# mitenjain/nanopore

Hardware: AMD Instinct MI355X
Metric: DP cells/sec (banded pair-HMM realign: forward + backward + posterior per cell) (higher is better)
Workload: dtype f32

## Files before the change

### nanopore_amd/csrc/npr_device.h

```cpp
#pragma once
#include <cstdint>

#include "npr_internal.h"
#include "npr_band.h"

namespace npr {

struct Task {
    int64_t x_off;
    int64_t y_off;
    int64_t band_off;
    int64_t pair_off;
    int32_t lX, lY;
    int32_t D;
    int32_t pair_cap;
    int32_t flags;
    int32_t model;
    int32_t xs, ys;
    int32_t read;
    int32_t cells_pad;
    int64_t ctl_off;
    int64_t tile_off;
    int64_t rowmask_off;
};

struct Stripe {
    int32_t X;
    int32_t K;
    int32_t df, dl;
    uint32_t row0;
    int32_t pad[3];
};

struct TaskOut {
    float tot_m;
    int32_t tot_e;
    float btot_m;
    int32_t btot_e;
    int32_t npairs;
    int32_t status;
};

struct KernelArgs {
    const Task *tasks;
    TaskOut *outs;
    int32_t *queue;
    int32_t ntasks;
    const DevModel *models;
    const uint8_t *seq;
    const int32_t *lo;
    const int32_t *n;
    const uint32_t *coff;
    const Stripe *stripes;
    const uint32_t *rowmask;
    unsigned long long *prof;
    const int64_t *region;
    const uint32_t *ctl;
    char *F;
    int64_t slot_stride;
    int32_t slot_base;
    int32_t *px;
    int32_t *py;
    float *pp;
    float threshold;
    int32_t wcap;
    float *Bv;
    int32_t *Be;
    float *ring;
    float *Fx;
    double *em_T;
    double *em_E;
};

constexpr int EM_BINS = 32;

struct CompactArgs {
    const Task *tasks;
    const TaskOut *outs;
    const int64_t *dst_off;
    int32_t ntasks;
    const int32_t *px;
    const int32_t *py;
    const float *pp;
    int32_t *cx;
    int32_t *cy;
    float *cp;
};

int launch_generic(const KernelArgs &a, int grid, int threads, size_t lds_bytes, bool dense, bool global_ring, void *stream);
int launch_em(const KernelArgs &a, int grid, size_t lds_bytes, bool global_ring, void *stream);
size_t em_extra_lds_bytes();
int launch_compact(const CompactArgs &a, void *stream);
int launch_stair(const KernelArgs &a, int R, int grid, void *stream);
int launch_wide(const KernelArgs &a, int R, int NW, int grid, void *stream);
int launch_em_stair(const KernelArgs &a, int R, int grid, void *stream);
size_t em_stair_lds_bytes();
struct MeaArgs {
    const Task *tasks;
    const TaskOut *outs;
    int32_t ntasks, n_reads;
    const int32_t *px, *py;
    const float *pp;
    const int64_t *rx_off;
    const int64_t *ry_off;
    const int64_t *rp_off;
    int32_t *cnt, *start, *colsum;
    int32_t *sx, *sy, *sq, *back;
    int32_t *kx, *ky, *kq, *kback;
    int4 *vrec;
    int32_t *kept;
    const int32_t *np, *poff, *pboff, *lane_read, *lane_piece;
    int32_t *pb, *pbest;
    int32_t n_pieces;
    int32_t *best_who;
    int32_t *read_flag;
    double gap_gamma, match_gamma;
    int32_t ring;
    const int32_t *order;
    const int32_t *read_first, *read_ntasks, *task_of;
    int32_t sort_lds_bytes;
    int32_t sort_threads;
    int32_t any_global_sort;
    const int64_t *cnt_off;
    int32_t ring_only;
    int32_t *ops_tmp;
    const int64_t *ot_off;
    int32_t *n_ops, *chain_len;
    int64_t *chain_mass;
    uint32_t *ops_dense;
    const int64_t *od_off;
    int32_t *max_run;
    uint16_t *ops_dense16;
};
int launch_tile(const KernelArgs &a, int R, int NW, int grid, void *stream, bool flat = false);
size_t tile_lds_bytes(int nw);
int64_t tile_scratch_cells(int64_t rows, int R);
struct PlanSeg {
    int64_t point_first;
    int64_t band_off;
    int32_t pieces, lX, lY, pad;
};
struct SegSummary {
    int64_t cells;
    int64_t generic_cells;
    int32_t max_width;
    int32_t bad;
    int32_t rough;
    int32_t pad;
};
constexpr int kSchedClasses = 7;
constexpr int kSchedR[kSchedClasses] = {1, 2, 4, 2, 2, 4, 4};
constexpr int kSchedNW[kSchedClasses] = {1, 1, 1, 4, 8, 8, 12};
struct PlanArgs {
    int32_t n_segs, fixed_mode, width;
    const PlanPoint *points;
    const PlanSeg *segs;
    int32_t *lo, *n;
    SegSummary *summary;
};
struct SchedArgs {
    int32_t n_segs;
    const PlanSeg *segs;
    const SegSummary *summary;
    const int32_t *lo, *n;
    const int64_t *ctl_off;
    const uint32_t *cand;
    uint32_t *ctl;
    int32_t *cls;
    int64_t *cells;
};
struct StripeArgs {
    int32_t count, R;
    const int32_t *seg_index;
    const PlanSeg *segs;
    const SegSummary *summary;
    const int32_t *lo, *n;
    const int64_t *tile_off;
    Stripe *stripes;
    int64_t *rows;
};
struct CoffArgs {
    int32_t n_segs;
    const PlanSeg *segs;
    const int32_t *n;
    uint32_t *coff;
};
int launch_plan_bands(const PlanArgs &a, void *stream);
template <int R>
NPR_HD constexpr uint32_t row_bias() { return R == 4 ? 2048u : 1024u; }
NPR_HD constexpr bool stair_fits(int64_t rows, int slots) { return rows * slots < (int64_t(1) << 29) - 512; }
// ... 228 lines not shown
```

### nanopore_amd/csrc/npr_finish.cpp

```cpp
#include "npr_api_internal.h"

namespace npr_impl {

static int32_t grow_pinned(npr_ctx *ctx, void *&p, size_t &have, size_t bytes, const char *what) {
    if (bytes <= have) return NPR_OK;
    if (p) (void)hipHostFree(p);
    p = nullptr, have = 0;
    const hipError_t e = hipHostMalloc(&p, bytes + bytes / 4, hipHostMallocDefault);
    if (e != hipSuccess) return fail(ctx, NPR_ERR_NOMEM, what, e);
    have = bytes + bytes / 4;
    return NPR_OK;
}
int32_t grow_pin_pairs(npr_ctx *ctx, size_t bytes, const char *what) { return grow_pinned(ctx, ctx->pin_pairs, ctx->pin_pairs_bytes, bytes, what); }
int32_t grow_pin_stage(npr_ctx *ctx, size_t bytes, const char *what) { return grow_pinned(ctx, ctx->pin_stage, ctx->pin_stage_bytes, bytes, what); }

int32_t fetch_pieced(npr_ctx *ctx, const PiecedFetch &f) {
    if (f.count <= 0) return NPR_OK;
    const int32_t grown = grow_pin_pairs(ctx, f.elem * static_cast<size_t>(f.count), f.what_pin);
    if (grown != NPR_OK) return grown;
    constexpr int64_t kMaxPieces = 48;
    const int64_t pieces = std::min(kMaxPieces, (f.count + f.per_piece - 1) / f.per_piece);
    const int64_t piece = ((f.count + pieces - 1) / pieces + f.round_to - 1) / f.round_to * f.round_to;
    while (static_cast<int64_t>(ctx->ops_events.size()) < pieces) {
        hipEvent_t ev;
// ... 142 lines not shown
                if (len > 0) out[0] = static_cast<int32_t>(x), out[1] = static_cast<int32_t>(y), out[2] = len, out += 3;
                x += len, y += len;
            } else if (op == NPR_OP_I) {
                y += len;
            } else {
                x += len;
            }
        }
    });
    tm.lap("runs");
    DevBuf<int64_t> d_run_off;
    DevBuf<int32_t> d_runs;
    hipError_t e;
    if ((e = d_run_off.alloc_from(ctx, n + 1)) != hipSuccess || (e = b->d_rs_gx_off.alloc_from(ctx, n + 1)) != hipSuccess ||
        (e = d_runs.alloc_from(ctx, std::max<size_t>(3 * static_cast<size_t>(run_off[n]), 1))) != hipSuccess ||
        (e = b->d_rs_gy.alloc_from(ctx, std::max<int64_t>(gx_off[n], 1))) != hipSuccess)
        return fail(ctx, NPR_ERR_NOMEM, "npr_batch_create: hipMalloc (rescore tables)", e);
    HIP_TRY(ctx, hipMemcpyAsync(d_run_off.p, run_off.data(), sizeof(int64_t) * (n + 1), hipMemcpyHostToDevice, ctx->stream));
    HIP_TRY(ctx, hipMemcpyAsync(b->d_rs_gx_off.p, gx_off.data(), sizeof(int64_t) * (n + 1), hipMemcpyHostToDevice, ctx->stream));
    if (run_bytes) HIP_TRY(ctx, hipMemcpyAsync(d_runs.p, runs, run_bytes, hipMemcpyHostToDevice, ctx->stream));
    HIP_TRY(ctx, hipMemsetAsync(b->d_rs_gy.p, 0xff, sizeof(int32_t) * std::max<int64_t>(gx_off[n], 1), ctx->stream));
    RescoreArgs ra{static_cast<int32_t>(n), 0, d_run_off.p, d_runs.p, b->d_rs_gx_off.p, b->d_rs_gy.p, nullptr, nullptr, nullptr, nullptr, nullptr, nullptr, shift};
    const int rc = launch_rescore_table(ra, ctx->stream);
    if (rc != 0) return fail(ctx, NPR_ERR_HIP, "k_rescore_table launch", static_cast<hipError_t>(rc));
    HIP_TRY(ctx, hipStreamSynchronize(ctx->stream));
    tm.lap("table");
    b->rs_shift = shift, b->rs_staged = true;
    return NPR_OK;
}

int32_t rescore_sum(npr_batch *b, std::vector<double> &score) {
    npr_ctx *ctx = b->ctx;
    const int64_t n = b->n_reads, ntasks = static_cast<int64_t>(b->tasks.size());
    DevBuf<unsigned long long> d_sum;
    hipError_t e;
    if ((e = d_sum.alloc_from(ctx, n)) != hipSuccess) return fail(ctx, NPR_ERR_NOMEM, "npr_batch_finish: hipMalloc (rescore sums)", e);
    HIP_TRY(ctx, hipMemsetAsync(d_sum.p, 0, sizeof(unsigned long long) * n, ctx->stream));
    RescoreArgs ra{static_cast<int32_t>(n), static_cast<int32_t>(ntasks), nullptr, nullptr, b->d_rs_gx_off.p, b->d_rs_gy.p, b->d_tasks.p, b->d_outs.p,
                   b->d_px.p, b->d_py.p, b->d_pp.p, d_sum.p, b->rs_shift};
    const int rc = launch_rescore_sum(ra, ctx->stream);
    if (rc != 0) return fail(ctx, NPR_ERR_HIP, "k_rescore_sum launch", static_cast<hipError_t>(rc));
    std::vector<unsigned long long> sum(n);
    HIP_TRY(ctx, hipMemcpyAsync(sum.data(), d_sum.p, sizeof(unsigned long long) * n, hipMemcpyDeviceToHost, ctx->stream));
    HIP_TRY(ctx, hipStreamSynchronize(ctx->stream));
    score.assign(n, 0.0);
    for (int64_t i = 0; i < n; ++i)
        if (b->rs_columns[i] > 0) score[i] = std::ldexp(static_cast<double>(sum[i]), -b->rs_shift) / static_cast<double>(b->rs_columns[i]);
    return NPR_OK;
}


constexpr int32_t kHostStage = 1;

struct MeaPlan {
    int64_t n = 0, total = 0, n_pieces = 0;
    size_t ntask_map = 0, n_cnt = 1;
    int64_t span = 0;
    bool sort_in_lds = true;
    std::vector<int64_t> offs;
    int64_t stride() const { return n + 1; }
    int64_t *arr(int k) { return offs.data() + k * stride(); }
    int64_t cols() const { return offs[2 * stride() - 1]; }
    int64_t ops_bound() const { return offs[4 * stride() - 1]; }
    std::vector<int32_t> order;
    std::vector<int32_t> pieces_head;
};

constexpr int64_t kOffArrays = 5, kSortedArrays = 8, kSmallArrays = 6, kVrecWords = 4;

MeaPlan plan_mea(const npr_batch *b) {
    MeaPlan p;
    const int64_t n = p.n = b->n_reads;
    p.offs.assign(kOffArrays * p.stride(), 0);
    int64_t *const rx = p.arr(0), *const ry = p.arr(1), *const rp = p.arr(2), *const ot = p.arr(3), *const cnt_off = p.arr(4);
    for (int64_t i = 0; i < n; ++i) {
        const bool ok = b->results[i].status == NPR_OK;
        const int64_t lX = ok ? b->ref_len[i] : 0, lY = ok ? b->read_len[i] : 0, np = ok ? b->pair_off[i + 1] - b->pair_off[i] : 0;
        rx[i + 1] = rx[i] + lX + 1;
        ry[i + 1] = ry[i] + lY;
        rp[i + 1] = rp[i] + np;
        ot[i + 1] = ot[i] + 3 * std::min({np, lX, lY}) + 2;
    }
    p.total = rp[n];
    const int64_t lds_span = b->ctx->opt[NPR_OPT_MEA_GLOBAL_SORT] != 0 ? 0 : 16 * 1024;
    int64_t cnt_total = 0;
    for (int64_t i = 0; i < n; ++i) {
        const int64_t sp = std::max(rx[i + 1] - rx[i], ry[i + 1] - ry[i]);
        cnt_off[i] = -1;
        if (sp <= lds_span) p.span = std::max(p.span, sp);
        else cnt_off[i] = cnt_total, cnt_total += rx[i + 1] - rx[i];
    }
    cnt_off[n] = -1;
    p.sort_in_lds = cnt_total == 0;
    p.n_cnt = p.sort_in_lds ? 1 : static_cast<size_t>(cnt_total);
    p.ntask_map = b->task_of.size();
    p.order.resize(n);
    std::iota(p.order.begin(), p.order.end(), 0);
    std::stable_sort(p.order.begin(), p.order.end(), [&](int32_t x, int32_t y) { return rp[x + 1] - rp[x] > rp[y + 1] - rp[y]; });
    constexpr int64_t kMaxPieces = 64, kLanesWanted = 64 * 5 * 256;
    const int64_t kPiecePairs = std::min<int64_t>(2048, std::max<int64_t>(128, p.total / kLanesWanted));
    std::vector<int32_t> np(n);
    for (int64_t i = 0; i < n; ++i) np[i] = static_cast<int32_t>(std::min(kMaxPieces, std::max<int64_t>(1, (rp[i + 1] - rp[i] + kPiecePairs - 1) / kPiecePairs))), p.n_pieces += np[i];
    p.pieces_head.resize(3 * n + 2 * p.n_pieces);
    int32_t *const t_np = p.pieces_head.data(), *const t_poff = t_np + n, *const t_pboff = t_poff + n, *const t_lr = t_pboff + n, *const t_lp = t_lr + p.n_pieces;
    int64_t at = 0;
    for (int64_t k = 0; k < n; ++k) {
        const int32_t r = p.order[k];
        t_np[r] = np[r], t_poff[r] = static_cast<int32_t>(at), t_pboff[r] = static_cast<int32_t>(at + k);
        for (int32_t j = 0; j < np[r]; ++j) t_lr[at + j] = r, t_lp[at + j] = j;
        at += np[r];
    }
    return p;
}

static_assert(kSortedArrays % kVrecWords == 0, "vrec starts on a 16-byte boundary of m.sorted (the arena's tables start 256-byte aligned)");
inline int64_t sorted_stride(const MeaPlan &p) { return p.total + 1; }

template <typename F>
hipError_t for_each_table(MeaScratch &m, const MeaPlan &p, F &&f) {
    hipError_t e = hipSuccess;
    auto one = [&](auto &buf, int64_t count) {
        if (e == hipSuccess) e = f(buf, static_cast<size_t>(count));
    };
    one(m.off, kOffArrays * p.stride());
    one(m.mass, p.n);
    one(m.od, p.n + 1);
    one(m.cnt, p.n_cnt);
    one(m.start, p.n_cnt);
    one(m.col, p.cols() + 1);
    one(m.sorted, kSortedArrays * sorted_stride(p) + kVrecWords * (p.total + 2));
    one(m.small, kSmallArrays * p.n);
    one(m.tmp, 2 * p.ops_bound());
    one(m.map, 3 * p.n + p.ntask_map);
    one(m.dense, p.ops_bound());
    one(m.pieces, 4 * p.n_pieces + 4 * p.n);
    return e;
}

inline size_t table_align(size_t bytes) { return (bytes + 255) & ~size_t(255); }

int32_t carve_tables(npr_ctx *ctx, MeaScratch &m, const MeaPlan &p, size_t need) {
    if (poison_byte() >= 0) {
        HIP_TRY(ctx, hipStreamSynchronize(ctx->stream));
        poison(ctx->arena->F, need);
    }
    char *cur = ctx->arena->F;
    (void)for_each_table(m, p, [&](auto &buf, size_t count) {
        using T = std::remove_pointer_t<decltype(buf.p)>;
        buf.borrow(reinterpret_cast<T *>(cur), count);
        cur += table_align(sizeof(T) * count);
        return hipSuccess;
    });
    return NPR_OK;
}

int32_t obtain_tables(npr_ctx *ctx, MeaScratch &m, const MeaPlan &p, std::unique_lock<std::mutex> &arena_lock) {
    size_t need = 0;
    (void)for_each_table(m, p, [&](auto &buf, size_t count) { return need += table_align(sizeof(*buf.p) * count), hipSuccess; });
    auto arena_fits = [&] { return ctx->arena->F && need <= static_cast<size_t>(ctx->arena->cells.load()) * 8; };
    const bool fits = arena_fits();
    if (!ctx->overlap && fits) return carve_tables(ctx, m, p, need);
    if (for_each_table(m, p, [](auto &buf, size_t count) { return buf.reserve(count); }) == hipSuccess) return NPR_OK;
    (void)hipGetLastError();
    if (!(ctx->overlap && fits)) return kHostStage;
    (void)for_each_table(m, p, [](auto &buf, size_t) { return buf.release(), hipSuccess; });
    ctx->cache_flush();
    arena_lock.lock();
    if (!arena_fits()) return kHostStage;
    ++ctx->arena->epoch;
    return carve_tables(ctx, m, p, need);
}

int32_t upload_tables(npr_batch *b, const MeaPlan &p, MeaScratch &m, MeaArgs &a) {
    npr_ctx *ctx = b->ctx;
    const int64_t n = p.n, P = p.n_pieces, so = p.stride(), ss = sorted_stride(p);
    a.tasks = b->d_tasks.p, a.outs = b->d_outs.p, a.ntasks = static_cast<int32_t>(b->tasks.size()), a.n_reads = static_cast<int32_t>(n);
    a.px = b->d_px.p, a.py = b->d_py.p, a.pp = b->d_pp.p;
    a.rx_off = m.off.p, a.ry_off = m.off.p + so, a.rp_off = m.off.p + 2 * so, a.ot_off = m.off.p + 3 * so, a.cnt_off = m.off.p + 4 * so;
    a.cnt = m.cnt.p, a.start = m.start.p, a.colsum = m.col.p;
    a.sx = m.sorted.p, a.sy = m.sorted.p + ss, a.sq = m.sorted.p + 2 * ss, a.back = m.sorted.p + 3 * ss;
    a.kx = m.sorted.p + 4 * ss, a.ky = m.sorted.p + 5 * ss, a.kq = m.sorted.p + 6 * ss, a.kback = m.sorted.p + 7 * ss;
    a.vrec = reinterpret_cast<int4 *>(m.sorted.p + kSortedArrays * ss);
    a.best_who = m.small.p, a.read_flag = m.small.p + n, a.n_ops = m.small.p + 2 * n, a.chain_len = m.small.p + 3 * n, a.kept = m.small.p + 4 * n, a.max_run = m.small.p + 5 * n;
    a.chain_mass = m.mass.p;
    int32_t *const read_first = m.map.p, *const read_ntasks = read_first + n, *const task_of = read_ntasks + n, *const order = task_of + p.ntask_map;
    a.read_first = read_first, a.read_ntasks = read_ntasks, a.task_of = task_of, a.order = order;
    int32_t *const lanes = m.pieces.p + 3 * n;
    a.np = m.pieces.p, a.poff = m.pieces.p + n, a.pboff = m.pieces.p + 2 * n, a.lane_read = lanes, a.lane_piece = lanes + P, a.pbest = lanes + 2 * P, a.pb = lanes + 3 * P;
    a.n_pieces = static_cast<int32_t>(P);
    a.ops_tmp = m.tmp.p, a.od_off = m.od.p;
    a.gap_gamma = b->params.gap_gamma, a.match_gamma = b->params.match_gamma;
    a.ring = 8192;
    a.ring_only = ctx->opt[NPR_OPT_MEA_RING_ONLY] != 0 ? 1 : 0;
    a.sort_lds_bytes = static_cast<int32_t>(4 * p.span);
    a.sort_threads = ctx->overlap == 1 ? 512 : 0;
    a.any_global_sort = p.sort_in_lds ? 0 : 1;
    HIP_TRY(ctx, hipMemcpyAsync(read_first, b->read_first_task.data(), sizeof(int32_t) * n, hipMemcpyHostToDevice, ctx->stream));
    HIP_TRY(ctx, hipMemcpyAsync(read_ntasks, b->read_ntasks.data(), sizeof(int32_t) * n, hipMemcpyHostToDevice, ctx->stream));
    HIP_TRY(ctx, hipMemcpyAsync(task_of, b->task_of.data(), sizeof(int32_t) * p.ntask_map, hipMemcpyHostToDevice, ctx->stream));
    HIP_TRY(ctx, hipMemcpyAsync(order, p.order.data(), sizeof(int32_t) * n, hipMemcpyHostToDevice, ctx->stream));
    HIP_TRY(ctx, hipMemcpyAsync(m.pieces.p, p.pieces_head.data(), sizeof(int32_t) * p.pieces_head.size(), hipMemcpyHostToDevice, ctx->stream));
    HIP_TRY(ctx, hipMemcpyAsync(m.off.p, p.offs.data(), m.off.bytes(), hipMemcpyHostToDevice, ctx->stream));
    HIP_TRY(ctx, hipMemsetAsync(m.small.p, 0, m.small.bytes(), ctx->stream));
    return NPR_OK;
}

int32_t run_chain(npr_ctx *ctx, const MeaArgs &a, MeaScratch &m, std::vector<int32_t> &small, std::vector<int64_t> &mass) {
    int rc = launch_mea_sort(a, ctx->stream);
    if (rc == 0) rc = launch_mea_chain(a, ctx->stream);
    if (rc != 0) return fail(ctx, NPR_ERR_HIP, "MEA kernel launch", static_cast<hipError_t>(rc));
    small.resize(m.small.count), mass.resize(m.mass.count);
    HIP_TRY(ctx, hipMemcpyAsync(small.data(), m.small.p, m.small.bytes(), hipMemcpyDeviceToHost, ctx->stream));
    HIP_TRY(ctx, hipMemcpyAsync(mass.data(), m.mass.p, m.mass.bytes(), hipMemcpyDeviceToHost, ctx->stream));
    HIP_TRY(ctx, hipStreamSynchronize(ctx->stream));
    return NPR_OK;
}

int32_t collect_results(npr_batch *b, const std::vector<int32_t> &small, const std::vector<int64_t> &mass, int32_t &longest) {
    const int64_t n = b->n_reads;
    const int32_t *flag = small.data() + n, *nops = small.data() + 2 * n, *clen = small.data() + 3 * n, *max_run = small.data() + 5 * n;
    for (int64_t i = 0; i < n; ++i)
        if (b->results[i].status == NPR_OK && flag[i] == NPR_ERR_CAPACITY) return kHostStage;
    std::vector<int64_t> &od = b->ops_off;
    od.assign(n + 1, 0);
    longest = 0;
    for (int64_t i = 0; i < n; ++i) {
        npr_read_result &r = b->results[i];
        if (r.status == NPR_OK && flag[i] != 0) r.status = flag[i];
        const int64_t k = r.status == NPR_OK ? nops[i] : 0;
        od[i + 1] = od[i] + k;
        if (k) longest = std::max(longest, max_run[i]);
        r.n_ops = k;
        r.score = (r.status == NPR_OK && clen[i] > 0) ? static_cast<double>(mass[i]) / (static_cast<double>(clen[i]) * PROB_ONE) : 0.0;
    }
    b->ops_words = 2 * od[n];
    return NPR_OK;
}

int32_t gather_ops(npr_batch *b, MeaScratch &m, MeaArgs &a, uint16_t *dense16) {
    npr_ctx *ctx = b->ctx;
    HIP_TRY(ctx, hipMemcpyAsync(m.od.p, b->ops_off.data(), m.od.bytes(), hipMemcpyHostToDevice, ctx->stream));
    if (b->ops_off[b->n_reads] == 0) return NPR_OK;
    a.ops_dense = m.dense.p, a.ops_dense16 = dense16;
    const int rc = launch_mea_gather(a, ctx->stream);
    return rc == 0 ? NPR_OK : fail(ctx, NPR_ERR_HIP, "k_mea_gather launch", static_cast<hipError_t>(rc));
}
void words_stay_on_device(npr_batch *b, const MeaScratch &m) { b->dev_ops = m.dense.p, b->dev_od = m.od.p, b->dev_ops_epoch = b->ctx->arena->epoch; }

int32_t hand_over_words(npr_batch *b, MeaScratch &m, MeaArgs &a, int32_t longest) {
    npr_ctx *ctx = b->ctx;
    const int64_t words = b->ops_off[b->n_reads];
    b->have_pairs_form = false, b->have_packed_form = true;
    if (words > b->packed_cap) ctx->take_packed(words, b->packed, b->packed_cap);
    if (words > b->packed_cap) {
        b->packed.reset(new uint32_t[words + words / 8]);
        b->packed_cap = words + words / 8;
    }
    if (words == 0) return NPR_OK;
    const bool narrow = longest < (1 << 14) && ctx->opt[NPR_OPT_MEA_WIDE_OPS] == 0 &&
                        sizeof(uint16_t) * static_cast<size_t>(words) <= m.sorted.bytes();
    int32_t rc = gather_ops(b, m, a, narrow ? reinterpret_cast<uint16_t *>(m.sorted.p) : nullptr);
    if (rc != NPR_OK) return rc;
    PiecedFetch f{m.dense.p, b->packed.get(), words, sizeof(uint32_t), int64_t(1) << 20, 64, nullptr, "npr_batch_finish: hipHostMalloc", "npr_batch_finish: D2H of the ops"};
    f.move = [](void *dst, const void *pin, int64_t lo, int64_t hi) {
        std::memcpy(static_cast<uint32_t *>(dst) + lo, static_cast<const uint32_t *>(pin) + lo, sizeof(uint32_t) * static_cast<size_t>(hi - lo));
// ... 340 lines not shown
```

### nanopore_amd/csrc/npr_mea.hip

```cpp
#include <hip/hip_runtime.h>

#include "npr_device.h"

namespace npr {
namespace {

constexpr int64_t P1 = PROB_ONE;
constexpr int WAVE = 64;
constexpr int SORT_THREADS = 1024;

__device__ __forceinline__ int rdlane(int v, int j) { return __builtin_amdgcn_readlane(v, j); }
__device__ __forceinline__ int64_t rdlane64(int64_t v, int j) {
    const int lo = __builtin_amdgcn_readlane(static_cast<int>(v), j);
    const int hi = __builtin_amdgcn_readlane(static_cast<int>(v >> 32), j);
    return (static_cast<int64_t>(hi) << 32) | static_cast<uint32_t>(lo);
}
__device__ __forceinline__ void wave_sync() {
    __builtin_amdgcn_fence(__ATOMIC_RELEASE, "wavefront");
    __builtin_amdgcn_wave_barrier();
    __builtin_amdgcn_fence(__ATOMIC_ACQUIRE, "wavefront");
}
__device__ __forceinline__ bool beats(int64_t s, int w, int64_t os, int ow) { return s > os || (s == os && w > ow); }

__device__ __forceinline__ int mea_task_pairs(const TaskOut &o, const Task &tk) { return o.status == NPR_OK ? min(max(o.npairs, 0), tk.pair_cap) : 0; }
__device__ __forceinline__ bool mea_is_posterior(float p) { return p >= 0.f && p <= 1.0f + 0x1p-10f; }

__global__ void __launch_bounds__(256) k_mea_zero(MeaArgs a) {
    const int r = blockIdx.x;
    const int64_t c0 = a.cnt_off[r];
    if (c0 < 0) return;
    const int nx = static_cast<int>(a.rx_off[r + 1] - a.rx_off[r]), ny = static_cast<int>(a.ry_off[r + 1] - a.ry_off[r]);
    for (int i = threadIdx.x; i < nx; i += blockDim.x) a.cnt[c0 + i] = 0;
    for (int i = threadIdx.x; i < ny; i += blockDim.x) a.colsum[a.ry_off[r] + i] = 0;
}

__global__ void __launch_bounds__(256) k_mea_count(MeaArgs a) {
    for (int t = blockIdx.x; t < a.ntasks; t += gridDim.x) {
        const Task &tk = a.tasks[t];
        const int n = mea_task_pairs(a.outs[t], tk);
        const int r = tk.read;
        const int64_t rx = a.cnt_off[r], ry = a.ry_off[r];
        if (rx < 0) continue;
        const int lX = static_cast<int>(a.rx_off[r + 1] - a.rx_off[r]) - 1, lY = static_cast<int>(a.ry_off[r + 1] - ry);
        for (int i = threadIdx.x; i < n; i += blockDim.x) {
            const int x = a.px[tk.pair_off + i], y = a.py[tk.pair_off + i];
            if (x < 0 || x >= lX || y < 0 || y >= lY || !mea_is_posterior(a.pp[tk.pair_off + i])) {
                a.read_flag[r] = NPR_ERR_INVALID;
                continue;
            }
            const int q = static_cast<int>(floor(static_cast<double>(a.pp[tk.pair_off + i]) * static_cast<double>(P1)));
            atomicAdd(a.cnt + rx + x, 1);
            atomicAdd(a.colsum + ry + y, q);
        }
    }
}

__global__ void __launch_bounds__(256) k_mea_scan(MeaArgs a) {
    __shared__ int wsum[4];
    const int r = blockIdx.x, tid = threadIdx.x, lane = tid & 63, wv = tid >> 6;
    const int64_t rx = a.cnt_off[r];
    if (rx < 0) return;
    const int n = static_cast<int>(a.rx_off[r + 1] - a.rx_off[r]);
    int carry = 0;
    for (int base = 0; base < n; base += 256) {
        const int i = base + tid;
        const int v = i < n ? a.cnt[rx + i] : 0;
        int s = v;
        for (int o = 1; o < WAVE; o <<= 1) {
            const int t = __shfl_up(s, o);
            if (lane >= o) s += t;
        }
        if (lane == WAVE - 1) wsum[wv] = s;
        __syncthreads();
        int before = 0, total = 0;
        for (int k = 0; k < 4; ++k) before += k < wv ? wsum[k] : 0, total += wsum[k];
        if (i < n) a.start[rx + i] = carry + before + s - v;
        carry += total;
        __syncthreads();
    }
}

__global__ void __launch_bounds__(256) k_mea_scatter(MeaArgs a) {
    for (int t = blockIdx.x; t < a.ntasks; t += gridDim.x) {
        const Task &tk = a.tasks[t];
        const int n = mea_task_pairs(a.outs[t], tk);
        const int r = tk.read;
        const int64_t rx = a.cnt_off[r], rp = a.rp_off[r];
        if (rx < 0) continue;
        const int lX = static_cast<int>(a.rx_off[r + 1] - a.rx_off[r]) - 1, lY = static_cast<int>(a.ry_off[r + 1] - a.ry_off[r]);
        for (int i = threadIdx.x; i < n; i += blockDim.x) {
            const int x = a.px[tk.pair_off + i], y = a.py[tk.pair_off + i];
            if (x < 0 || x >= lX || y < 0 || y >= lY || !mea_is_posterior(a.pp[tk.pair_off + i])) continue;
            const int q = static_cast<int>(floor(static_cast<double>(a.pp[tk.pair_off + i]) * static_cast<double>(P1)));
            const int64_t pos = rp + a.start[rx + x] + (atomicSub(a.cnt + rx + x, 1) - 1);
            a.sx[pos] = x, a.sy[pos] = y, a.sq[pos] = q;
        }
    }
}

__global__ void __launch_bounds__(SORT_THREADS) k_mea_sort_lds(MeaArgs a) {
    extern __shared__ int h[];
    __shared__ int wsum[SORT_THREADS / WAVE];
    const int r = a.order[blockIdx.x], tid = threadIdx.x, lane = tid & 63, wv = tid >> 6;
    const int nthreads = static_cast<int>(blockDim.x);
    const int64_t rx = a.rx_off[r], ry = a.ry_off[r], rp = a.rp_off[r];
    const int lX = static_cast<int>(a.rx_off[r + 1] - rx) - 1, lY = static_cast<int>(a.ry_off[r + 1] - ry);
    if (a.rp_off[r + 1] == rp || a.cnt_off[r] >= 0) return;
    const int ft = a.read_first[r], nt = a.read_ntasks[r];
    int bad = 0;
    auto for_pairs = [&](auto f) {
        for (int s = 0; s < nt; ++s) {
            const int t = a.task_of[ft + s];
            const Task &tk = a.tasks[t];
            const int n = mea_task_pairs(a.outs[t], tk);
            for (int i = tid; i < n; i += nthreads) {
                const int x = a.px[tk.pair_off + i], y = a.py[tk.pair_off + i];
                if (x < 0 || x >= lX || y < 0 || y >= lY || !mea_is_posterior(a.pp[tk.pair_off + i])) {
                    bad = 1;
                    continue;
                }
                f(x, y, static_cast<int>(floor(static_cast<double>(a.pp[tk.pair_off + i]) * static_cast<double>(P1))));
            }
        }
    };
    for (int i = tid; i < lY; i += nthreads) h[i] = 0;
    __syncthreads();
    for_pairs([&](int, int y, int q) { atomicAdd(&h[y], q); });
    __syncthreads();
    for (int i = tid; i < lY; i += nthreads) a.colsum[ry + i] = h[i];
    __syncthreads();
    for (int i = tid; i <= lX; i += nthreads) h[i] = 0;
    __syncthreads();
    for_pairs([&](int x, int, int) { atomicAdd(&h[x], 1); });
    __syncthreads();
    int carry = 0;
    for (int base = 0; base <= lX; base += nthreads) {
        const int i = base + tid;
        const int v = i <= lX ? h[i] : 0;
        int sc = v;
        for (int o = 1; o < WAVE; o <<= 1) {
            const int t = __shfl_up(sc, o);
            if (lane >= o) sc += t;
        }
        if (lane == WAVE - 1) wsum[wv] = sc;
        __syncthreads();
        int before = 0, total = 0;
        for (int k = 0; k < nthreads / WAVE; ++k) before += k < wv ? wsum[k] : 0, total += wsum[k];
        if (i <= lX) h[i] = carry + before + sc - v;
        carry += total;
        __syncthreads();
    }
    for_pairs([&](int x, int y, int q) {
        const int64_t pos = rp + atomicAdd(&h[x], 1);
        a.sx[pos] = x, a.sy[pos] = y, a.sq[pos] = q;
    });
    if (bad) a.read_flag[r] = NPR_ERR_INVALID;
}

constexpr int MEA_RETRY = 1;

struct Chunk {
    int valid;
    uint64_t ends;
    uint64_t keep;
    int y, q;
    int64_t w;
    int who;
};
__device__ __forceinline__ Chunk prep_chunk(const MeaArgs &a, int *sx, int *sy, int *sq, int64_t ry, int base, int n, int lane,
                                            int64_t floor_w, int64_t *tw, int *ty, int *tq) {
    Chunk c;
    const int pos = base + lane;
    const bool in = pos < n;
    const int x = in ? sx[pos] : -1, xn = pos + 1 < n ? sx[pos + 1] : -2;
    int y = in ? sy[pos] : 0, q = in ? sq[pos] : 0;
    const uint64_t ends = __ballot(in && x != xn);
    c.valid = ends ? 64 - __builtin_clzll(ends) : 0;
    c.ends = ends, c.keep = 0, c.y = 0, c.q = 0, c.w = 0;
    if (!ends) return c;
    const bool act = lane < c.valid;
    const uint64_t starts = (ends << 1) | 1ull;
    const int gfirst = 63 - __builtin_clzll(starts & (lane == 63 ? ~0ull : ((2ull << lane) - 1)));
    const int gend = act ? lane + __builtin_ctzll(ends >> lane) : lane;
    const int gsize = gend - gfirst + 1;
    int rank = 0, rowsum = q;
    for (int o = 1; __any(act && o < gsize); ++o) {
        const int lo = lane - o, hi = lane + o;
        const int yl = __shfl(y, lo & 63), ql = __shfl(q, lo & 63), yh = __shfl(y, hi & 63), qh = __shfl(q, hi & 63);
        if (lo >= gfirst) rank += yl < y ? 1 : 0, rowsum += ql;
        if (hi <= gend) rank += yh < y ? 1 : 0, rowsum += qh;
    }
    const int colsum = act ? a.colsum[ry + y] : 0;
    const int64_t gap = max(P1 - rowsum, int64_t(0)) + max(P1 - colsum, int64_t(0));
    const int64_t w0 = q - static_cast<int64_t>(floor(a.gap_gamma * static_cast<double>(gap)));
    wave_sync();
    if (act) {
        const int to = gend - rank;
        tw[to] = w0, ty[to] = y, tq[to] = q;
    }
    wave_sync();
    c.w = tw[lane], c.y = ty[lane], c.q = tq[lane];
    c.keep = __ballot(act && c.w > floor_w);
    c.who = gfirst + gend - lane;
    if (act) sy[base + c.who] = c.y, sq[base + c.who] = c.q;
    return c;
}

constexpr int WEIGH_CHUNK = 128;
constexpr int WEIGH_RING = 512;
constexpr int WEIGH_HALO = 64;
__device__ __forceinline__ int64_t pair_weight(int q, int rowsum, int colsum, double gap_gamma) {
    const int64_t gap = max(P1 - rowsum, int64_t(0)) + max(P1 - colsum, int64_t(0));
    return q - static_cast<int64_t>(floor(gap_gamma * static_cast<double>(gap)));
}
__global__ void __launch_bounds__(WAVE) k_mea_weigh(MeaArgs a) {
    __shared__ int X[WEIGH_RING], Y[WEIGH_RING], Q[WEIGH_RING], C[WEIGH_RING];
    const int r = a.order[blockIdx.x], lane = threadIdx.x;
    const int64_t rp = a.rp_off[r], ry = a.ry_off[r];
    const int n = a.read_flag[r] ? 0 : static_cast<int>(a.rp_off[r + 1] - rp);
    const int *const sx = a.sx + rp, *const sy = a.sy + rp, *const sq = a.sq + rp;
    const int *const col = a.colsum + ry;
    const int64_t floor_w = static_cast<int64_t>(floor(a.match_gamma * static_cast<double>(P1)));
    constexpr int RM = WEIGH_RING - 1;
    const int nc = (n + WEIGH_CHUNK - 1) / WEIGH_CHUNK;
    int giveup = 0;
    int fx[2], fy[2], fq[2];
    auto fetch = [&](int chunk) {
#pragma unroll
        for (int h = 0; h < 2; ++h) {
            const int j = chunk * WEIGH_CHUNK + h * WAVE + lane;
            const bool ok = j < n;
            fx[h] = ok ? sx[j] : -1, fy[h] = ok ? sy[j] : 0, fq[h] = ok ? sq[j] : 0;
        }
    };
    auto stage = [&](int chunk) {
        int fc[2];
#pragma unroll
        for (int h = 0; h < 2; ++h) fc[h] = fx[h] >= 0 ? col[fy[h]] : 0;
#pragma unroll
        for (int h = 0; h < 2; ++h) {
            const int k = (chunk * WEIGH_CHUNK + h * WAVE + lane) & RM;
            X[k] = fx[h], Y[k] = fy[h], Q[k] = fq[h], C[k] = fc[h];
        }
    };
    for (int k = lane; k < WEIGH_CHUNK; k += WAVE) X[(-WEIGH_CHUNK + k) & RM] = -2;
    if (nc > 0) {
        fetch(0);
        stage(0);
        fetch(1);
    }
    int carry = 0;
    for (int c = 0; c < nc; ++c) {
        stage(c + 1);
        fetch(c + 2);
        wave_sync();
        int keep[2], below[2], above[2], before[2], xs[2], ys[2], qs[2];
        int64_t ws[2];
#pragma unroll
        for (int h = 0; h < 2; ++h) {
            const int i = c * WEIGH_CHUNK + h * WAVE + lane, me = i & RM;
            const bool in = i < n;
            const int x = X[me], y = Y[me], q = Q[me];
            int gs = i, ge = i, rowsum = q;
            if (in) {
                while (gs > i - WEIGH_HALO && X[(gs - 1) & RM] == x) rowsum += Q[(--gs) & RM];
                while (ge < i + WEIGH_HALO && X[(ge + 1) & RM] == x) rowsum += Q[(++ge) & RM];
                if (gs == i - WEIGH_HALO || ge == i + WEIGH_HALO) giveup = 1;
            }
            const int64_t w = in ? pair_weight(q, rowsum, C[me], a.gap_gamma) : 0;
            keep[h] = in && w > floor_w;
            before[h] = below[h] = above[h] = 0;
            if (keep[h])
                for (int j = gs; j <= ge; ++j) {
                    const int k = j & RM;
                    if (j != i && pair_weight(Q[k], rowsum, C[k], a.gap_gamma) > floor_w) before[h] += j < i, below[h] += Y[k] < y, above[h] += Y[k] > y;
                }
            xs[h] = x, ys[h] = y, qs[h] = q, ws[h] = w;
        }
        int sc0 = keep[0], sc1 = keep[1];
        for (int o = 1; o < WAVE; o <<= 1) {
            const int t0 = __shfl_up(sc0, o), t1 = __shfl_up(sc1, o);
            if (lane >= o) sc0 += t0, sc1 += t1;
        }
        const int tot0 = __shfl(sc0, WAVE - 1), tot1 = __shfl(sc1, WAVE - 1);
        const int ex[2] = {sc0 - keep[0], tot0 + sc1 - keep[1]};
#pragma unroll
        for (int h = 0; h < 2; ++h)
            if (keep[h]) {
                const int64_t g0 = rp + carry + ex[h] - before[h];
                const int64_t id = g0 + below[h], at = g0 + above[h];
                a.kx[id] = xs[h], a.ky[id] = ys[h], a.kq[id] = qs[h];
                a.vrec[at] = make_int4(ys[h], static_cast<int>(ws[h]), static_cast<int>(id - rp), 0);
            }
        carry += tot0 + tot1;
        wave_sync();
    }
    giveup = __any(giveup);
    if (lane == 0) {
        a.kept[r] = giveup ? -1 : carry;
        if (giveup && a.read_flag[r] == 0) a.read_flag[r] = MEA_RETRY;
    }
}

constexpr int MEA_MAX_PIECES = 64;
__global__ void __launch_bounds__(WAVE) k_mea_cuts(MeaArgs a) {
    __shared__ int PM[MEA_MAX_PIECES][WAVE];
    const int r = a.order[blockIdx.x], lane = threadIdx.x;
    const int np = a.np[r];
    int *const pb = a.pb + a.pboff[r];
    const int m = a.read_flag[r] == 0 ? max(a.kept[r], 0) : 0;
    const int64_t rp = a.rp_off[r];
    const int *const kx = a.kx + rp, *const ky = a.ky + rp;
    const int nb = (m + WAVE - 1) / WAVE;
    if (np <= 1 || nb < 2) {
        for (int k = lane; k <= np; k += WAVE) pb[k] = k == 0 ? 0 : m;
        return;
    }
    auto target = [&](int j) { return static_cast<int>(static_cast<int64_t>(j) * nb / np); };
    constexpr int NEG = -(1 << 30), POS = 1 << 30;
    int rm = NEG, j = 1;
    for (int b = 0; b < nb && j < np; ++b) {
        const int idx = b * WAVE + lane;
        const int v = idx < m ? ky[idx] : NEG;
        if (target(j) == b) {
            int before = rm;
            for (int o = 32; o; o >>= 1) before = max(before, __shfl_xor(before, o));
            int sc = v;
            for (int o = 1; o < WAVE; o <<= 1) {
                const int t = __shfl_up(sc, o);
                if (lane >= o) sc = max(sc, t);
            }
            const int pm = max(sc, before);
            while (j < np && target(j) == b) PM[j][lane] = pm, ++j;
        }
        rm = max(rm, v);
    }
    int rn = POS;
    j = np - 1;
    for (int b = nb - 1; b >= 0 && j >= 1; --b) {
        const int idx = b * WAVE + lane;
        const int v = idx < m ? ky[idx] : POS;
        if (target(j) == b) {
            int after = rn;
            for (int o = 32; o; o >>= 1) after = min(after, __shfl_xor(after, o));
            int sc = v;
            for (int o = 1; o < WAVE; o <<= 1) {
                const int t = __shfl_down(sc, o);
                if (lane + o < WAVE) sc = min(sc, t);
            }
            int ex = __shfl_down(sc, 1);
            if (lane == WAVE - 1) ex = POS;
            const int sm = min(ex, after);
            const bool can = idx + 1 < m && kx[idx] != kx[idx + 1];
            while (j >= 1 && target(j) == b) {
                const uint64_t ok = __ballot(can && PM[j][lane] < sm);
                int at = -1;
                if (ok >> 32) at = 32 + __builtin_ctzll(ok >> 32);
                else if (ok) at = 63 - __builtin_clzll(ok);
                if (lane == 0) pb[j] = at < 0 ? -1 : b * WAVE + at + 1;
                --j;
// ... 204 lines not shown
    int64_t mass = 0;
    bool broken = false;
    const bool alive = a.read_flag[r] == 0;
    int piece = by_id ? __builtin_amdgcn_readfirstlane(a.np[r]) : 1;
    const int *const pbest = a.pbest + (by_id ? a.poff[r] : 0);
    while (piece-- > 0) {
    int i = !alive ? -1 : __builtin_amdgcn_readfirstlane(by_id ? pbest[piece] : a.best_who[r]);
    while (i >= 0) {
        const int cb = max(i - (WAVE - 1), 0), idx = min(cb + lane, i);
        const int vb = back[idx], vx = sx[idx], vy = sy[idx], vq = sq[idx];
        const int rel = (vb - cb) & (WAVE - 1);
        const bool diag = vb >= cb && __shfl(vx, rel) == vx - 1 && __shfl(vy, rel) == vy - 1;
        int nxt = diag ? rel : lane, val = diag ? vq : 0;
#pragma unroll
        for (int k = 0; k < 6; ++k) {
            val += __shfl(val, nxt);
            nxt = __shfl(nxt, nxt);
        }
        while (i >= cb) {
            const int l = i - cb, h = rdlane(nxt, l);
            const int x = rdlane(vx, l), y = rdlane(vy, l), hx = rdlane(vx, h), hy = rdlane(vy, h);
            emit(NPR_OP_I, cy - y - 1);
            emit(NPR_OP_D, cx - x - 1);
            emit(NPR_OP_M, x - hx + 1);
            cx = hx, cy = hy, mass += rdlane(val, l) + rdlane(vq, h), len += x - hx + 1;
            const int to = rdlane(vb, h);
            if (to >= i) {
                broken = true;
                i = -1;
                break;
            }
            i = to;
        }
    }
    if (broken) break;
    }
    emit(NPR_OP_I, cy);
    emit(NPR_OP_D, cx);
    if (hop >= 0 && p > lo) {
        --p;
        if (lane == 0) *p = make_int2(hop, hlen);
        longest = max(longest, hlen);
    }
    if (lane == 0) {
        if (broken) a.read_flag[r] = NPR_ERR_INVALID;
        a.max_run[r] = longest;
        a.n_ops[r] = broken ? 0 : static_cast<int>(reinterpret_cast<int2 *>(a.ops_tmp) + a.ot_off[r + 1] - p);
        a.chain_len[r] = len;
        a.chain_mass[r] = mass;
    }
}

__global__ void __launch_bounds__(256) k_mea_gather(MeaArgs a) {
    for (int r = blockIdx.x; r < a.n_reads; r += gridDim.x) {
        const int n = static_cast<int>(a.od_off[r + 1] - a.od_off[r]);
        const int2 *src = reinterpret_cast<const int2 *>(a.ops_tmp) + a.ot_off[r + 1] - a.n_ops[r];
        uint32_t *dst = a.ops_dense + a.od_off[r];
        uint16_t *const dst16 = a.ops_dense16 ? a.ops_dense16 + a.od_off[r] : nullptr;
        for (int i = threadIdx.x; i < n; i += blockDim.x) {
            const uint32_t w = static_cast<uint32_t>(src[i].y) << 2 | static_cast<uint32_t>(src[i].x);
            dst[i] = w;
            if (dst16) dst16[i] = static_cast<uint16_t>(w);
        }
    }
}

}

size_t mea_chain_lds_bytes(int ring) { return static_cast<size_t>(ring) * 12 + WAVE * (8 + 4 + 4); }

int launch_mea_sort(const MeaArgs &a, void *stream) {
    hipStream_t s = static_cast<hipStream_t>(stream);
    if (a.sort_lds_bytes > 0) {
        const hipError_t e = hipFuncSetAttribute(reinterpret_cast<const void *>(k_mea_sort_lds), hipFuncAttributeMaxDynamicSharedMemorySize, a.sort_lds_bytes);
        if (e != hipSuccess) return static_cast<int>(e);
        hipLaunchKernelGGL(k_mea_sort_lds, dim3(a.n_reads), dim3(a.sort_threads >= WAVE && a.sort_threads < SORT_THREADS ? a.sort_threads & ~(WAVE - 1) : SORT_THREADS), a.sort_lds_bytes, s, a);
    }
    if (a.any_global_sort) {
        const int tg = a.ntasks < 8192 ? (a.ntasks > 0 ? a.ntasks : 1) : 8192;
        hipLaunchKernelGGL(k_mea_zero, dim3(a.n_reads), dim3(256), 0, s, a);
        hipLaunchKernelGGL(k_mea_count, dim3(tg), dim3(256), 0, s, a);
        hipLaunchKernelGGL(k_mea_scan, dim3(a.n_reads), dim3(256), 0, s, a);
        hipLaunchKernelGGL(k_mea_scatter, dim3(tg), dim3(256), 0, s, a);
    }
    return static_cast<int>(hipGetLastError());
}

int launch_mea_chain(const MeaArgs &a, void *stream) {
    hipStream_t s = static_cast<hipStream_t>(stream);
    const size_t lds = mea_chain_lds_bytes(a.ring);
    const hipError_t e = hipFuncSetAttribute(reinterpret_cast<const void *>(k_mea_chain), hipFuncAttributeMaxDynamicSharedMemorySize, static_cast<int>(lds));
    if (e != hipSuccess) return static_cast<int>(e);
    const int lanes_lds = LWIN * WAVE * static_cast<int>(sizeof(int64_t));
    const hipError_t e2 = hipFuncSetAttribute(reinterpret_cast<const void *>(k_mea_chain_lanes), hipFuncAttributeMaxDynamicSharedMemorySize, lanes_lds);
    if (e2 != hipSuccess) return static_cast<int>(e2);
    hipLaunchKernelGGL(k_mea_weigh, dim3(a.n_reads), dim3(WAVE), 0, s, a);
    hipLaunchKernelGGL(k_mea_cuts, dim3(a.n_reads), dim3(WAVE), 0, s, a);
    hipLaunchKernelGGL(k_mea_chain_lanes, dim3((a.n_pieces + WAVE - 1) / WAVE), dim3(WAVE), lanes_lds, s, a);
    hipLaunchKernelGGL(k_mea_chain, dim3(a.n_reads < 512 ? (a.n_reads > 0 ? a.n_reads : 1) : 512), dim3(WAVE), lds, s, a);
    hipLaunchKernelGGL(k_mea_trace, dim3(a.n_reads), dim3(WAVE), 0, s, a);
    return static_cast<int>(hipGetLastError());
}

int launch_mea_gather(const MeaArgs &a, void *stream) {
    const int g = a.n_reads < 8192 ? a.n_reads : 8192;
    hipLaunchKernelGGL(k_mea_gather, dim3(g), dim3(256), 0, static_cast<hipStream_t>(stream), a);
    return static_cast<int>(hipGetLastError());
}

}
```

Before: 374.1 billion.

## Fuse MEA weight computation into LDS sort and cache pairs in registers

```diff
diff --git a/nanopore_amd/csrc/npr_device.h b/nanopore_amd/csrc/npr_device.h
--- a/nanopore_amd/csrc/npr_device.h
+++ b/nanopore_amd/csrc/npr_device.h
@@ -95,6 +95,7 @@
 int launch_wide(const KernelArgs &a, int R, int NW, int grid, void *stream);
 int launch_em_stair(const KernelArgs &a, int R, int grid, void *stream);
 size_t em_stair_lds_bytes();
+constexpr int kMeaSortLdsSpan = 16 * 1024;
 struct MeaArgs {
     const Task *tasks;
     const TaskOut *outs;
@@ -106,6 +107,7 @@
     const int64_t *rp_off;
     int32_t *cnt, *start, *colsum;
     int32_t *sx, *sy, *sq, *back;
+    int32_t *sw;
     int32_t *kx, *ky, *kq, *kback;
     int4 *vrec;
     int32_t *kept;
diff --git a/nanopore_amd/csrc/npr_finish.cpp b/nanopore_amd/csrc/npr_finish.cpp
--- a/nanopore_amd/csrc/npr_finish.cpp
+++ b/nanopore_amd/csrc/npr_finish.cpp
@@ -248,12 +248,12 @@
         ot[i + 1] = ot[i] + 3 * std::min({np, lX, lY}) + 2;
     }
     p.total = rp[n];
-    const int64_t lds_span = b->ctx->opt[NPR_OPT_MEA_GLOBAL_SORT] != 0 ? 0 : 16 * 1024;
+    const int64_t lds_span = b->ctx->opt[NPR_OPT_MEA_GLOBAL_SORT] != 0 ? 0 : kMeaSortLdsSpan;
     int64_t cnt_total = 0;
     for (int64_t i = 0; i < n; ++i) {
         const int64_t sp = std::max(rx[i + 1] - rx[i], ry[i + 1] - ry[i]);
         cnt_off[i] = -1;
-        if (sp <= lds_span) p.span = std::max(p.span, sp);
+        if (sp <= lds_span) p.span = std::max(p.span, (rx[i + 1] - rx[i]) + (ry[i + 1] - ry[i]));
         else cnt_off[i] = cnt_total, cnt_total += rx[i + 1] - rx[i];
     }
     cnt_off[n] = -1;
@@ -294,7 +294,7 @@
     one(m.cnt, p.n_cnt);
     one(m.start, p.n_cnt);
     one(m.col, p.cols() + 1);
-    one(m.sorted, kSortedArrays * sorted_stride(p) + kVrecWords * (p.total + 2));
+    one(m.sorted, kSortedArrays * sorted_stride(p) + kVrecWords * (p.total + 2) + sorted_stride(p));
     one(m.small, kSmallArrays * p.n);
     one(m.tmp, 2 * p.ops_bound());
     one(m.map, 3 * p.n + p.ntask_map);
@@ -347,6 +347,7 @@
     a.sx = m.sorted.p, a.sy = m.sorted.p + ss, a.sq = m.sorted.p + 2 * ss, a.back = m.sorted.p + 3 * ss;
     a.kx = m.sorted.p + 4 * ss, a.ky = m.sorted.p + 5 * ss, a.kq = m.sorted.p + 6 * ss, a.kback = m.sorted.p + 7 * ss;
     a.vrec = reinterpret_cast<int4 *>(m.sorted.p + kSortedArrays * ss);
+    a.sw = m.sorted.p + kSortedArrays * ss + kVrecWords * (p.total + 2);
     a.best_who = m.small.p, a.read_flag = m.small.p + n, a.n_ops = m.small.p + 2 * n, a.chain_len = m.small.p + 3 * n, a.kept = m.small.p + 4 * n, a.max_run = m.small.p + 5 * n;
     a.chain_mass = m.mass.p;
     int32_t *const read_first = m.map.p, *const read_ntasks = read_first + n, *const task_of = read_ntasks + n, *const order = task_of + p.ntask_map;
diff --git a/nanopore_amd/csrc/npr_mea.hip b/nanopore_amd/csrc/npr_mea.hip
--- a/nanopore_amd/csrc/npr_mea.hip
+++ b/nanopore_amd/csrc/npr_mea.hip
@@ -98,6 +98,32 @@
     }
 }
 
+__device__ __forceinline__ int64_t pair_weight(int q, int rowsum, int colsum, double gap_gamma) {
+    const int64_t gap = max(P1 - rowsum, int64_t(0)) + max(P1 - colsum, int64_t(0));
+    return q - static_cast<int64_t>(floor(gap_gamma * static_cast<double>(gap)));
+}
+__device__ __forceinline__ int stored_weight(int q, int rowsum, int colsum, double gap_gamma) {
+    return static_cast<int>(max(pair_weight(q, rowsum, colsum, gap_gamma), static_cast<int64_t>(INT32_MIN)));
+}
+__device__ __forceinline__ int mea_quantum(float p) { return static_cast<int>(floor(static_cast<double>(p) * static_cast<double>(P1))); }
+
+__global__ void __launch_bounds__(256) k_mea_weight_sorted(MeaArgs a) {
+    const int r = blockIdx.x;
+    const int64_t rx = a.cnt_off[r], ry = a.ry_off[r], rp = a.rp_off[r];
+    if (rx < 0 || a.read_flag[r]) return;
+    const int n = static_cast<int>(a.rp_off[r + 1] - rp);
+    const int lX = static_cast<int>(a.rx_off[r + 1] - a.rx_off[r]) - 1, lY = static_cast<int>(a.ry_off[r + 1] - ry);
+    for (int i = threadIdx.x; i < n; i += blockDim.x) {
+        const int x = a.sx[rp + i], y = a.sy[rp + i];
+        if (x < 0 || x >= lX || y < 0 || y >= lY) continue;
+        int rowsum = 0;
+        for (int j = max(a.start[rx + x], 0); j < min(a.start[rx + x + 1], n); ++j) rowsum += a.sq[rp + j];
+        a.sw[rp + i] = stored_weight(a.sq[rp + i], rowsum, a.colsum[ry + y], a.gap_gamma);
+    }
+}
+
+constexpr int SORT_BUDGET = 22;
+static_assert(kMeaSortLdsSpan <= (1 << 16), "k_mea_sort_lds packs (x, y) into one word");
 __global__ void __launch_bounds__(SORT_THREADS) k_mea_sort_lds(MeaArgs a) {
     extern __shared__ int h[];
     __shared__ int wsum[SORT_THREADS / WAVE];
@@ -106,37 +132,84 @@
     const int64_t rx = a.rx_off[r], ry = a.ry_off[r], rp = a.rp_off[r];
     const int lX = static_cast<int>(a.rx_off[r + 1] - rx) - 1, lY = static_cast<int>(a.ry_off[r + 1] - ry);
     if (a.rp_off[r + 1] == rp || a.cnt_off[r] >= 0) return;
+    int *const cnt = h, *const col = cnt + lX + 1;
+    const int slots = static_cast<int>(a.rp_off[r + 1] - rp);
     const int ft = a.read_first[r], nt = a.read_ntasks[r];
-    int bad = 0;
-    auto for_pairs = [&](auto f) {
+    const int budget = nthreads * SORT_BUDGET;
+    int bad = 0, total = 0;
+    for (int s = 0; s < nt; ++s) {
+        const int t = a.task_of[ft + s];
+        total += mea_task_pairs(a.outs[t], a.tasks[t]);
+    }
+    auto for_overflow = [&](auto f) {
+        int first = 0;
         for (int s = 0; s < nt; ++s) {
             const int t = a.task_of[ft + s];
             const Task &tk = a.tasks[t];
             const int n = mea_task_pairs(a.outs[t], tk);
-            for (int i = tid; i < n; i += nthreads) {
+            for (int i = max(budget - first, 0) + tid; i < n; i += nthreads) {
                 const int x = a.px[tk.pair_off + i], y = a.py[tk.pair_off + i];
-                if (x < 0 || x >= lX || y < 0 || y >= lY || !mea_is_posterior(a.pp[tk.pair_off + i])) {
+                const float p = a.pp[tk.pair_off + i];
+                if (x < 0 || x >= lX || y < 0 || y >= lY || !mea_is_posterior(p)) {
                     bad = 1;
                     continue;
                 }
-                f(x, y, static_cast<int>(floor(static_cast<double>(a.pp[tk.pair_off + i]) * static_cast<double>(P1))));
-            }
+                f(x, y, mea_quantum(p));
+            }
+            first += n;
         }
     };
-    for (int i = tid; i < lY; i += nthreads) h[i] = 0;
+    int vx[SORT_BUDGET], vy[SORT_BUDGET];
+    float vp[SORT_BUDGET];
+    {
+        int64_t where[SORT_BUDGET];
+        int s = -1, first = 0, n = 0;
+        int64_t at = 0;
+#pragma unroll
+        for (int k = 0; k < SORT_BUDGET; ++k) {
+            const int g = k * nthreads + tid;
+            where[k] = -1;
+            if (g < total) {
+                while (g >= first + n) {
+                    const int t = a.task_of[ft + ++s];
+                    first += n, n = mea_task_pairs(a.outs[t], a.tasks[t]), at = a.tasks[t].pair_off;
+                }
+                where[k] = at + (g - first);
+            }
+        }
+#pragma unroll
+        for (int k = 0; k < SORT_BUDGET; ++k) {
+            const bool have = where[k] >= 0;
+            vx[k] = have ? a.px[where[k]] : 0, vy[k] = have ? a.py[where[k]] : 0, vp[k] = have ? a.pp[where[k]] : 0.f;
+        }
+    }
+    for (int i = tid; i < lX + 1 + lY; i += nthreads) h[i] = 0;
     __syncthreads();
-    for_pairs([&](int, int y, int q) { atomicAdd(&h[y], q); });
+    if (total > budget) {
+        for_overflow([&](int x, int y, int q) { atomicAdd(&cnt[x], 1), atomicAdd(&col[y], q); });
+        __syncthreads();
+    }
+    int vxy[SORT_BUDGET], vq[SORT_BUDGET], vrank[SORT_BUDGET];
+#pragma unroll
+    for (int k = 0; k < SORT_BUDGET; ++k) {
+        const int x = vx[k], y = vy[k];
+        const bool have = k * nthreads + tid < total;
+        const bool ok = have && x >= 0 && x < lX && y >= 0 && y < lY && mea_is_posterior(vp[k]);
+        if (have && !ok) bad = 1;
+        vxy[k] = -1, vq[k] = 0, vrank[k] = 0;
+        if (ok) {
+            const int q = mea_quantum(vp[k]);
+            vxy[k] = x << 16 | y, vq[k] = q;
+            vrank[k] = atomicAdd(&cnt[x], 1);
+            atomicAdd(&col[y], q);
+        }
+    }
     __syncthreads();
-    for (int i = tid; i < lY; i += nthreads) a.colsum[ry + i] = h[i];
-    __syncthreads();
-    for (int i = tid; i <= lX; i += nthreads) h[i] = 0;
-    __syncthreads();
-    for_pairs([&](int x, int, int) { atomicAdd(&h[x], 1); });
-    __syncthreads();
+    for (int i = tid; i < lY; i += nthreads) a.colsum[ry + i] = col[i];
     int carry = 0;
     for (int base = 0; base <= lX; base += nthreads) {
         const int i = base + tid;
-        const int v = i <= lX ? h[i] : 0;
+        const int v = i <= lX ? cnt[i] : 0;
         int sc = v;
         for (int o = 1; o < WAVE; o <<= 1) {
             const int t = __shfl_up(sc, o);
@@ -144,16 +217,44 @@
         }
         if (lane == WAVE - 1) wsum[wv] = sc;
         __syncthreads();
-        int before = 0, total = 0;
-        for (int k = 0; k < nthreads / WAVE; ++k) before += k < wv ? wsum[k] : 0, total += wsum[k];
-        if (i <= lX) h[i] = carry + before + sc - v;
-        carry += total;
+        int before = 0, sum = 0;
+        for (int k = 0; k < nthreads / WAVE; ++k) before += k < wv ? wsum[k] : 0, sum += wsum[k];
+        if (i <= lX) cnt[i] = carry + before + sc - v;
+        carry += sum;
         __syncthreads();
     }
-    for_pairs([&](int x, int y, int q) {
-        const int64_t pos = rp + atomicAdd(&h[x], 1);
-        a.sx[pos] = x, a.sy[pos] = y, a.sq[pos] = q;
-    });
+#pragma unroll
+    for (int k = 0; k < SORT_BUDGET; ++k)
+        if (vxy[k] != -1) vrank[k] += cnt[vxy[k] >> 16];
+    if (total > budget) {
+        __syncthreads();
+        for_overflow([&](int x, int y, int q) {
+            const int64_t pos = rp + atomicAdd(&cnt[x], 1);
+            a.sx[pos] = x, a.sy[pos] = y, a.sq[pos] = q;
+        });
+    }
+    __syncthreads();
+    for (int i = tid; i <= lX; i += nthreads) cnt[i] = 0;
+    __syncthreads();
+#pragma unroll
+    for (int k = 0; k < SORT_BUDGET; ++k)
+        if (vxy[k] != -1) atomicAdd(&cnt[vxy[k] >> 16], vq[k]);
+    if (total > budget) for_overflow([&](int x, int, int q) { atomicAdd(&cnt[x], q); });
+    __syncthreads();
+#pragma unroll
+    for (int k = 0; k < SORT_BUDGET; ++k)
+        if (vxy[k] != -1) {
+            const int x = vxy[k] >> 16, y = vxy[k] & 0xffff;
+            const int64_t pos = rp + vrank[k];
+            a.sx[pos] = x, a.sy[pos] = y, a.sq[pos] = vq[k], a.sw[pos] = stored_weight(vq[k], cnt[x], col[y], a.gap_gamma);
+        }
+    if (total > budget) {
+        __syncthreads();
+        for (int i = tid; i < slots; i += nthreads) {
+            const int x = a.sx[rp + i], y = a.sy[rp + i];
+            if (x >= 0 && x < lX && y >= 0 && y < lY) a.sw[rp + i] = stored_weight(a.sq[rp + i], cnt[x], col[y], a.gap_gamma);
+        }
+    }
     if (bad) a.read_flag[r] = NPR_ERR_INVALID;
 }
 
@@ -209,38 +310,30 @@
 constexpr int WEIGH_CHUNK = 128;
 constexpr int WEIGH_RING = 512;
 constexpr int WEIGH_HALO = 64;
-__device__ __forceinline__ int64_t pair_weight(int q, int rowsum, int colsum, double gap_gamma) {
-    const int64_t gap = max(P1 - rowsum, int64_t(0)) + max(P1 - colsum, int64_t(0));
-    return q - static_cast<int64_t>(floor(gap_gamma * static_cast<double>(gap)));
-}
 __global__ void __launch_bounds__(WAVE) k_mea_weigh(MeaArgs a) {
-    __shared__ int X[WEIGH_RING], Y[WEIGH_RING], Q[WEIGH_RING], C[WEIGH_RING];
+    __shared__ int X[WEIGH_RING], Y[WEIGH_RING], Q[WEIGH_RING], W[WEIGH_RING];
     const int r = a.order[blockIdx.x], lane = threadIdx.x;
-    const int64_t rp = a.rp_off[r], ry = a.ry_off[r];
+    const int64_t rp = a.rp_off[r];
     const int n = a.read_flag[r] ? 0 : static_cast<int>(a.rp_off[r + 1] - rp);
-    const int *const sx = a.sx + rp, *const sy = a.sy + rp, *const sq = a.sq + rp;
-    const int *const col = a.colsum + ry;
+    const int *const sx = a.sx + rp, *const sy = a.sy + rp, *const sq = a.sq + rp, *const sw = a.sw + rp;
     const int64_t floor_w = static_cast<int64_t>(floor(a.match_gamma * static_cast<double>(P1)));
     constexpr int RM = WEIGH_RING - 1;
     const int nc = (n + WEIGH_CHUNK - 1) / WEIGH_CHUNK;
     int giveup = 0;
-    int fx[2], fy[2], fq[2];
+    int fx[2], fy[2], fq[2], fw[2];
     auto fetch = [&](int chunk) {
 #pragma unroll
         for (int h = 0; h < 2; ++h) {
             const int j = chunk * WEIGH_CHUNK + h * WAVE + lane;
             const bool ok = j < n;
-            fx[h] = ok ? sx[j] : -1, fy[h] = ok ? sy[j] : 0, fq[h] = ok ? sq[j] : 0;
+            fx[h] = ok ? sx[j] : -1, fy[h] = ok ? sy[j] : 0, fq[h] = ok ? sq[j] : 0, fw[h] = ok ? sw[j] : 0;
         }
     };
     auto stage = [&](int chunk) {
-        int fc[2];
-#pragma unroll
-        for (int h = 0; h < 2; ++h) fc[h] = fx[h] >= 0 ? col[fy[h]] : 0;
 #pragma unroll
         for (int h = 0; h < 2; ++h) {
             const int k = (chunk * WEIGH_CHUNK + h * WAVE + lane) & RM;
-            X[k] = fx[h], Y[k] = fy[h], Q[k] = fq[h], C[k] = fc[h];
+            X[k] = fx[h], Y[k] = fy[h], Q[k] = fq[h], W[k] = fw[h];
         }
     };
     for (int k = lane; k < WEIGH_CHUNK; k += WAVE) X[(-WEIGH_CHUNK + k) & RM] = -2;
@@ -254,28 +347,26 @@
         stage(c + 1);
         fetch(c + 2);
         wave_sync();
-        int keep[2], below[2], above[2], before[2], xs[2], ys[2], qs[2];
-        int64_t ws[2];
+        int keep[2], below[2], above[2], before[2], xs[2], ys[2], qs[2], ws[2];
 #pragma unroll
         for (int h = 0; h < 2; ++h) {
             const int i = c * WEIGH_CHUNK + h * WAVE + lane, me = i & RM;
             const bool in = i < n;
-            const int x = X[me], y = Y[me], q = Q[me];
-            int gs = i, ge = i, rowsum = q;
+            const int x = X[me], y = Y[me], w = W[me];
+            int gs = i, ge = i;
             if (in) {
-                while (gs > i - WEIGH_HALO && X[(gs - 1) & RM] == x) rowsum += Q[(--gs) & RM];
-                while (ge < i + WEIGH_HALO && X[(ge + 1) & RM] == x) rowsum += Q[(++ge) & RM];
+                while (gs > i - WEIGH_HALO && X[(gs - 1) & RM] == x) --gs;
+                while (ge < i + WEIGH_HALO && X[(ge + 1) & RM] == x) ++ge;
                 if (gs == i - WEIGH_HALO || ge == i + WEIGH_HALO) giveup = 1;
             }
-            const int64_t w = in ? pair_weight(q, rowsum, C[me], a.gap_gamma) : 0;
             keep[h] = in && w > floor_w;
             before[h] = below[h] = above[h] = 0;
             if (keep[h])
                 for (int j = gs; j <= ge; ++j) {
                     const int k = j & RM;
-                    if (j != i && pair_weight(Q[k], rowsum, C[k], a.gap_gamma) > floor_w) before[h] += j < i, below[h] += Y[k] < y, above[h] += Y[k] > y;
+                    if (j != i && W[k] > floor_w) before[h] += j < i, below[h] += Y[k] < y, above[h] += Y[k] > y;
                 }
-            xs[h] = x, ys[h] = y, qs[h] = q, ws[h] = w;
+            xs[h] = x, ys[h] = y, qs[h] = Q[me], ws[h] = w;
         }
         int sc0 = keep[0], sc1 = keep[1];
         for (int o = 1; o < WAVE; o <<= 1) {
@@ -646,6 +737,7 @@
         hipLaunchKernelGGL(k_mea_count, dim3(tg), dim3(256), 0, s, a);
         hipLaunchKernelGGL(k_mea_scan, dim3(a.n_reads), dim3(256), 0, s, a);
         hipLaunchKernelGGL(k_mea_scatter, dim3(tg), dim3(256), 0, s, a);
+        hipLaunchKernelGGL(k_mea_weight_sorted, dim3(a.n_reads), dim3(256), 0, s, a);
     }
     return static_cast<int>(hipGetLastError());
 }
```

After: 383.6 billion, median of 6. +2.5%, better.
